# zkHubHQ/distributed-groth16

Measured on AMD Instinct MI355X. Metric: groth16_constraints_per_sec, higher is better.
Workload: dtype u32; 1 GPU; BN254 Groth16 prove from the matrices, synthetic R1CS with 2^20 - 2 constraints (3 nonzeros per row of A and B), 2^20 wires, 2 instance variables; r, s != 0 (R1CS x witness + 6 NTTs of 2^20 + 4 G1 MSMs + 1 G2 MSM); proving key RESIDENT as window tables (built once per key outside the timed region); curve=bn254, log_domain=20, parallelism=single GPU, key_table_bytes=6039807360, key_table_stride=1

## Files before the change

distributed-groth16_amd/csrc/ntt.hip:

```cpp
#include <cstdio>
#include <cstdlib>
#include "ctx.h"
#include "fp29.h"
#include "types.h"

namespace dg16 {

static void optional_table_skipped(const char* what, size_t bytes) {
  static const bool verbose = [] { const char* e = getenv("DG16_VERBOSE"); return e && atoi(e) != 0; }();
  if (verbose) fprintf(stderr, "[dg16] %s (%zu bytes) not built: hipMalloc failed; using the composed form\n", what, bytes);
}


constexpr unsigned kTileLog = 10;
constexpr unsigned kTile = 1u << kTileLog;
constexpr unsigned kMaxStepLog = 10;
constexpr unsigned kLoBits = 11;

template <class F>
struct StepArgs {
  const F* src[3];
  F* dst[3];
  unsigned log_n, s, log_a, log_b;
  unsigned last;
  unsigned log_n1, log_n2;
  const F* small;
  unsigned sm;
  const F* tw_lo;
  const F* tw_hi;
  unsigned lb;
  const F* tw_full;
  const F* post_full;
  const F* pre_lo;
  const F* pre_hi;
  const F* post_lo;
  const F* post_hi;
  unsigned plb;
  const F* scale;
  unsigned src_piece_log, dst_piece_log;
  size_t src_piece_stride, dst_piece_stride;
};

__device__ __forceinline__ unsigned bitrev(unsigned v, unsigned bits) {
  return bits ? (__brev(v) >> (32 - bits)) : 0;
}

constexpr int kNttBound = 48 * 64;
constexpr int kNttIn = 128;
constexpr int kNttFirstOut = 9 * 64;
constexpr int kNttStepGrowth = 6 * 64 + 32;
constexpr int kNttOddGrowth = 3 * 64 + 32;
static_assert(kNttFirstOut + (int)((kMaxStepLog - 2) / 2) * kNttStepGrowth + kNttOddGrowth <= kNttBound,
              "NTT tile bound: a pass of kMaxStepLog levels can exceed kNttBound");

template <class F>
__global__ void __launch_bounds__(256) ntt_step_kernel(StepArgs<F> p) {
  using P = typename F::Params;
  using T = RR<P>;
  constexpr int N = T::N;
  using El = Fe<P, kNttBound, 1>;
  using Tw = Fe<P, 64, 1>;
  __shared__ uint32_t tile_w[kTile * N];
  constexpr int NLW = T::NL;
  __shared__ uint32_t tw_w[(1u << (kMaxStepLog - 1)) * NLW];
  static_assert((1u << (kMaxStepLog - 2)) * N <= (1u << (kMaxStepLog - 1)) * NLW, "unpacked twiddles of the shorter steps fit");
  const unsigned tid = threadIdx.x;
  const unsigned s = p.s;
  const unsigned nj = 1u << s;
  const unsigned log_t = (p.log_n < kTileLog ? p.log_n : kTileLog) - s;
  const unsigned Tn = 1u << log_t;
  const unsigned elems = nj << log_t;
  const size_t tile_id = blockIdx.x;
  auto slot = [](unsigned e) { return (e ^ ((e >> 2) & 31u)) * (unsigned)N; };
  auto ld_tile = [&](unsigned i) {
    El v;
    const unsigned o = slot(i);
#pragma unroll
    for (int j = 0; j < N; j++) v.l[j] = tile_w[o + j];
    return v;
  };
  auto st_tile = [&](unsigned i, const El& v) {
    const unsigned o = slot(i);
#pragma unroll
    for (int j = 0; j < N; j++) tile_w[o + j] = v.l[j];
  };
  const bool tw_packed = p.s == kMaxStepLog;
  auto ld_tw = [&](unsigned i) {
    if (tw_packed) return fe_from_words<P>(&tw_w[i * NLW]);
    Tw v;
#pragma unroll
    for (int j = 0; j < N; j++) v.l[j] = tw_w[i * N + j];
    return v;
  };
  auto ld_packed = [&](const F* ptr) { return fe_from_words<P>(ptr->l); };

  size_t a = 0, b0 = 0, k1_0 = 0, k2 = 0;
  if (!p.last) {
    const unsigned tiles_per_a_log = p.log_b - log_t;
    a = tile_id >> tiles_per_a_log;
    b0 = (tile_id & (((size_t)1 << tiles_per_a_log) - 1)) << log_t;
  } else {
    const unsigned k1_tiles_log = p.log_n1 - log_t;
    k2 = tile_id >> k1_tiles_log;
    k1_0 = (tile_id & (((size_t)1 << k1_tiles_log) - 1)) << log_t;
  }

  if (s >= 1)
    for (unsigned t = tid; t < (nj >> 1); t += 256) {
      const F* w = p.small + ((size_t)t << (p.sm - s));
      if (tw_packed) {
#pragma unroll
        for (int j = 0; j < NLW; j++) tw_w[t * NLW + j] = w->l[j];
      } else {
        const Tw u = ld_packed(w);
#pragma unroll
        for (int j = 0; j < N; j++) tw_w[t * N + j] = u.l[j];
      }
    }

  for (unsigned idx = tid; idx < elems; idx += 256) {
    unsigned n, t;
    size_t g;
    if (!p.last) {
      t = idx & (Tn - 1);
      n = idx >> log_t;
      g = ((((a << s) + n) << p.log_b) + b0 + t);
    } else {
      n = idx & (nj - 1);
      t = idx >> s;
      g = ((((k1_0 + t) << p.log_n2) + k2) << s) + n;
    }
    const size_t gs = p.src_piece_stride ? (g >> p.src_piece_log) * p.src_piece_stride + (g & (((size_t)1 << p.src_piece_log) - 1)) : g;
    const Tw x = ld_packed(p.src[blockIdx.y] + gs);
    El v = x.template as<kNttBound, 1>();
    if (p.pre_lo) {
      const auto w = ld_packed(p.pre_lo + (g & ((1u << p.plb) - 1))) * ld_packed(p.pre_hi + (g >> p.plb));
      v = (x * w).template as<kNttBound, 1>();
    }
    st_tile((bitrev(n, s) << log_t) + t, v);
  }
  __syncthreads();

  unsigned lv = 1;
  if (s >= 2) {
    using In = Fe<P, kNttIn, 1>;
    const Tw w3 = ld_tw(1u << (s - 2));
    for (unsigned q = tid; q < (elems >> 2); q += 256) {
      const unsigned t = q & (Tn - 1), pi = q >> log_t;
      const unsigned ia = (pi << (2 + log_t)) + t;
      const In xa = ld_tile(ia).template unsafe_assume<kNttIn, 1>(), xb = ld_tile(ia + Tn).template unsafe_assume<kNttIn, 1>(),
               xc = ld_tile(ia + 2 * Tn).template unsafe_assume<kNttIn, 1>(), xd = ld_tile(ia + 3 * Tn).template unsafe_assume<kNttIn, 1>();
      const auto a1 = xa + xb;
      const auto b1 = xa - xb;
      const auto c1 = xc + xd;
      const auto te = (xc - xd) * w3;
      const auto o0 = a1 + c1;
      const auto o2 = a1 - c1;
      const auto o1 = b1 + te;
      const auto o3 = b1 - te;
      static_assert(decltype(o0)::Bound <= kNttFirstOut && decltype(o1)::Bound <= kNttFirstOut &&
                    decltype(o2)::Bound <= kNttFirstOut && decltype(o3)::Bound <= kNttFirstOut, "first radix-4 step bound");
      st_tile(ia, norm(o0).template as<kNttBound, 1>());
      st_tile(ia + 2 * Tn, norm(o2).template as<kNttBound, 1>());
      st_tile(ia + Tn, norm(o1).template as<kNttBound, 1>());
      st_tile(ia + 3 * Tn, norm(o3).template as<kNttBound, 1>());
    }
    __syncthreads();
    lv = 3;
  }
  for (; lv + 1 <= s; lv += 2) {
    const unsigned half = 1u << (lv - 1);
    const unsigned sh1 = s - lv, sh2 = s - lv - 1;
    for (unsigned q = tid; q < (elems >> 2); q += 256) {
      const unsigned t = q & (Tn - 1), pi = q >> log_t;
      const unsigned k = pi & (half - 1), blk = pi >> (lv - 1);
      const unsigned ia = ((((blk << (lv + 1)) + k)) << log_t) + t;
      const unsigned st = half << log_t;
      const El xa = ld_tile(ia), xb = ld_tile(ia + st), xc = ld_tile(ia + 2 * st), xd = ld_tile(ia + 3 * st);
      const Tw w1 = ld_tw(k << sh1);
      const auto tb = xb * w1;
      const auto td = xd * w1;
      const auto a1 = xa + tb;
      const auto b1 = xa - tb;
      const auto c1 = xc + td;
      const auto d1 = xc - td;
      const auto tc = c1 * ld_tw(k << sh2);
      const auto te = d1 * ld_tw((k + half) << sh2);
      const auto o0 = a1 + tc;
      const auto o2 = a1 - tc;
      const auto o1 = b1 + te;
      const auto o3 = b1 - te;
      static_assert(decltype(o0)::Bound - kNttBound <= kNttStepGrowth && decltype(o1)::Bound - kNttBound <= kNttStepGrowth &&
                    decltype(o2)::Bound - kNttBound <= kNttStepGrowth && decltype(o3)::Bound - kNttBound <= kNttStepGrowth,
                    "radix-4 step growth");
      st_tile(ia, norm(o0).template unsafe_assume<kNttBound, 1>());
      st_tile(ia + 2 * st, norm(o2).template unsafe_assume<kNttBound, 1>());
      st_tile(ia + st, norm(o1).template unsafe_assume<kNttBound, 1>());
      st_tile(ia + 3 * st, norm(o3).template unsafe_assume<kNttBound, 1>());
    }
    __syncthreads();
  }
  if (lv == s) {
    const unsigned half = 1u << (s - 1);
    for (unsigned q = tid; q < (elems >> 1); q += 256) {
      const unsigned t = q & (Tn - 1), k = q >> log_t;
      const unsigned i0 = (k << log_t) + t, i1 = i0 + (half << log_t);
      const El x = ld_tile(i0);
      const auto ty = ld_tile(i1) * ld_tw(k);
      const auto o0 = x + ty;
      const auto o1 = x - ty;
      static_assert(decltype(o0)::Bound - kNttBound <= kNttOddGrowth && decltype(o1)::Bound - kNttBound <= kNttOddGrowth,
                    "odd level growth");
      st_tile(i0, norm(o0).template unsafe_assume<kNttBound, 1>());
      st_tile(i1, norm(o1).template unsafe_assume<kNttBound, 1>());
    }
    __syncthreads();
  }

  for (unsigned idx = tid; idx < elems; idx += 256) {
    unsigned t = idx & (Tn - 1);
    unsigned k = idx >> log_t;
    const El v = ld_tile((k << log_t) + t);
    Fe<P, 64, 1> out;
    size_t g;
    if (!p.last) {
      size_t b = b0 + t;
      size_t e = (b * k) << p.log_a;
      if (p.tw_full) {
        if (e || p.scale) out = canon(v * ld_packed(p.tw_full + (((size_t)k << p.log_b) + b)));
        else out = canon(v);
      } else if (e) {
        const auto w = ld_packed(p.tw_lo + (e & ((1u << p.lb) - 1))) * ld_packed(p.tw_hi + (e >> p.lb));
        out = canon(v * w);
      } else if (p.scale) {
        out = canon(v * ld_packed(p.tw_hi));
      } else {
        out = canon(v);
      }
      g = ((((a << s) + k) << p.log_b) + b);
    } else {
      g = (k1_0 + t) + (k2 << p.log_n1) + ((size_t)k << (p.log_n1 + p.log_n2));
      if (p.post_full) {
        const auto w = ld_packed(p.post_full + g);
        if (p.scale) out = canon((v * ld_packed(p.scale)) * w);
        else out = canon(v * w);
      } else if (p.scale && p.post_lo) {
        const auto w = ld_packed(p.post_lo + (g & ((1u << p.plb) - 1))) * ld_packed(p.post_hi + (g >> p.plb));
        out = canon((v * ld_packed(p.scale)) * w);
      } else if (p.scale) {
        out = canon(v * ld_packed(p.scale));
      } else if (p.post_lo) {
        const auto w = ld_packed(p.post_lo + (g & ((1u << p.plb) - 1))) * ld_packed(p.post_hi + (g >> p.plb));
        out = canon(v * w);
      } else {
        out = canon(v);
      }
    }
    F o;
    fe_to_words<P>(out, o.l);
    if (p.dst_piece_stride) g = (g >> p.dst_piece_log) * p.dst_piece_stride + (g & (((size_t)1 << p.dst_piece_log) - 1));
    p.dst[blockIdx.y][g] = o;
  }
}

template <class F>
__global__ void to_internal_kernel(F* t, size_t count) {
  size_t j = (size_t)blockIdx.x * blockDim.x + threadIdx.x;
  if (j >= count) return;
  using P = typename F::Params;
  F c;
#pragma unroll
  for (int i = 0; i < F::NL; i++) c.l[i] = RR<P>::R_WORDS.v[i];
  t[j] = t[j] * c;
}
template <class F>
static void* internal_copy(hipStream_t s, const void* src, size_t count) {
  void* d = nullptr;
  DG_HIP(hipMalloc(&d, count * sizeof(F)));
  DG_HIP(hipMemcpyAsync(d, src, count * sizeof(F), hipMemcpyDeviceToDevice, s));
  hipLaunchKernelGGL(to_internal_kernel<F>, dim3((unsigned)((count + 255) / 256)), dim3(256), 0, s, (F*)d, count);
  return d;
}

template <class F>
__global__ void powers_kernel(F* out, size_t count, unsigned shift, const F* base_ptr,
                              unsigned root_log, int invert, const F* c_ptr) {
  size_t j = (size_t)blockIdx.x * blockDim.x + threadIdx.x;
  if (j >= count) return;
  F base;
  if (base_ptr) {
    base = *base_ptr;
  } else {
    F w;
#pragma unroll
    for (int i = 0; i < F::NL; i++) w.l[i] = F::Params::TWO_ADIC_ROOT[i];
    for (unsigned i = root_log; i < (unsigned)F::Params::TWO_ADICITY; i++) w = w.sqr();
    if (invert) {
      F acc = F::one(), sq = w;
      for (unsigned i = 0; i < root_log; i++) { acc = acc * sq; sq = sq.sqr(); }
      w = acc;
    }
    base = w;
  }
  F r = base.pow_u64((uint64_t)j << shift);
  if (c_ptr) r = r * *c_ptr;
  out[j] = r;
}

template <class F>
__global__ void n_inv_kernel(F* out, unsigned log_n) {
  F two = F::one() + F::one();
  F half = two.inv();
  *out = half.pow_u64(log_n);
}

struct Plan {
  unsigned nsteps;
  unsigned s[3];
};
static Plan make_plan(unsigned log_n) {
  Plan pl{};
  if (log_n <= kTileLog && log_n <= kMaxStepLog) {
    pl.nsteps = 1;
    pl.s[0] = log_n;
  } else if (log_n <= 2 * kMaxStepLog) {
    pl.nsteps = 2;
    pl.s[0] = log_n / 2;
    pl.s[1] = log_n - pl.s[0];
  } else {
    pl.nsteps = 3;
    pl.s[0] = log_n / 3;
    pl.s[1] = (log_n - pl.s[0]) / 2;
    pl.s[2] = log_n - pl.s[0] - pl.s[1];
  }
  return pl;
}

constexpr unsigned kFullTwiddleMaxLog = 24;
inline unsigned full_twiddle_min_log() {
  static const unsigned v = [] { const char* e = getenv("DG16_NTT_TABLE_MIN_LOG"); return e ? (unsigned)atoi(e) : 21u; }();
  return v;
}
template <class F>
__global__ void __launch_bounds__(256) full_twiddle_kernel(F* __restrict__ out, size_t count, unsigned log_a, unsigned log_b,
                                                            const F* __restrict__ lo, const F* __restrict__ hi, unsigned lb) {
  using P = typename F::Params;
  const size_t idx = (size_t)blockIdx.x * blockDim.x + threadIdx.x;
  if (idx >= count) return;
  const size_t k = idx >> log_b, b = idx & (((size_t)1 << log_b) - 1);
  const size_t e = (b * k) << log_a;
  const auto w = fe_from_words<P>(lo[e & (((size_t)1 << lb) - 1)].l) * fe_from_words<P>(hi[e >> lb].l);
  F o;
  fe_to_words<P>(canon(w), o.l);
  out[idx] = o;
}
template <class F>
__global__ void __launch_bounds__(256) flat_powers_kernel(F* __restrict__ out, size_t count, const F* __restrict__ lo,
                                                           const F* __restrict__ hi, unsigned lb) {
  using P = typename F::Params;
  const size_t o = (size_t)blockIdx.x * blockDim.x + threadIdx.x;
  if (o >= count) return;
  const auto w = fe_from_words<P>(lo[o & (((size_t)1 << lb) - 1)].l) * fe_from_words<P>(hi[o >> lb].l);
  F r;
  fe_to_words<P>(canon(w), r.l);
  out[o] = r;
}

template <class F>
static const TwiddleSet& get_twiddles(Call& k, int curve, unsigned log_n, int inverse) {
  std::lock_guard<std::mutex> g(k.ctx->mu);
  TwiddleKey key{curve, log_n, inverse};
  auto it = k.ctx->twiddles.find(key);
  if (it != k.ctx->twiddles.end()) return it->second;
  TwiddleSet ts;
  ts.lb = log_n < kLoBits ? log_n : kLoBits;
  ts.sm = log_n < kMaxStepLog ? (log_n ? log_n : 1) : kMaxStepLog;
  size_t nlo = (size_t)1 << ts.lb, nhi = (size_t)1 << (log_n - ts.lb), nsm = (size_t)1 << (ts.sm - 1);
  DG_HIP(hipMalloc(&ts.lo, nlo * sizeof(F)));
  DG_HIP(hipMalloc(&ts.hi, nhi * sizeof(F)));
  DG_HIP(hipMalloc(&ts.small, nsm * sizeof(F)));
  DG_HIP(hipMalloc(&ts.n_inv, sizeof(F)));
  hipStream_t s = k.s();
  hipLaunchKernelGGL(n_inv_kernel<F>, dim3(1), dim3(1), 0, s, (F*)ts.n_inv, log_n);
  hipLaunchKernelGGL(powers_kernel<F>, dim3((unsigned)((nlo + 255) / 256)), dim3(256), 0, s, (F*)ts.lo,
                     nlo, 0u, (const F*)nullptr, log_n, inverse, (const F*)nullptr);
  hipLaunchKernelGGL(powers_kernel<F>, dim3((unsigned)((nhi + 255) / 256)), dim3(256), 0, s, (F*)ts.hi,
                     nhi, ts.lb, (const F*)nullptr, log_n, inverse, (const F*)nullptr);
  if (inverse) {
    DG_HIP(hipMalloc(&ts.hi_scaled, nhi * sizeof(F)));
    hipLaunchKernelGGL(powers_kernel<F>, dim3((unsigned)((nhi + 255) / 256)), dim3(256), 0, s,
                       (F*)ts.hi_scaled, nhi, ts.lb, (const F*)nullptr, log_n, inverse,
                       (const F*)ts.n_inv);
  }
  hipLaunchKernelGGL(powers_kernel<F>, dim3((unsigned)((nsm + 255) / 256)), dim3(256), 0, s, (F*)ts.small,
                     nsm, log_n >= ts.sm ? log_n - ts.sm : 0, (const F*)nullptr, log_n ? log_n : 1, inverse,
                     (const F*)nullptr);
  ts.lo_i = internal_copy<F>(s, ts.lo, nlo);
  ts.hi_i = internal_copy<F>(s, ts.hi, nhi);
  if (inverse) ts.hi_scaled_i = internal_copy<F>(s, ts.hi_scaled, nhi);
  ts.small_i = internal_copy<F>(s, ts.small, nsm);
  ts.n_inv_i = internal_copy<F>(s, ts.n_inv, 1);
  {
    const Plan pl = make_plan(log_n);
    unsigned consumed = 0;
    for (unsigned j = 0; j + 1 < pl.nsteps && log_n <= kFullTwiddleMaxLog && log_n >= full_twiddle_min_log(); j++) {
      const size_t cnt = (size_t)1 << (log_n - consumed);
      if (hipMalloc(&ts.full[j], cnt * sizeof(F)) != hipSuccess) {
        (void)hipGetLastError();
        ts.full[j] = nullptr;
        optional_table_skipped("inter-step twiddle table", cnt * sizeof(F));
        consumed += pl.s[j];
        continue;
      }
      hipLaunchKernelGGL(full_twiddle_kernel<F>, dim3((unsigned)((cnt + 255) / 256)), dim3(256), 0, s, (F*)ts.full[j], cnt,
                         consumed, log_n - consumed - pl.s[j], (const F*)ts.lo_i,
                         (const F*)((inverse && j == 0) ? ts.hi_scaled_i : ts.hi_i), ts.lb);
      consumed += pl.s[j];
    }
  }
  DG_HIP(hipGetLastError());
  DG_HIP(hipStreamSynchronize(s));
  return k.ctx->twiddles.emplace(key, ts).first->second;
}

template <class F>
static void build_power_tables(Call& k, const F* g_dev, unsigned log_n, F* lo, F* hi, unsigned lb) {
  size_t nlo = (size_t)1 << lb, nhi = (size_t)1 << (log_n - lb);
  hipLaunchKernelGGL(powers_kernel<F>, dim3((unsigned)((nlo + 255) / 256)), dim3(256), 0, k.s(), lo, nlo, 0u,
                     g_dev, 0u, 0, (const F*)nullptr);
  hipLaunchKernelGGL(powers_kernel<F>, dim3((unsigned)((nhi + 255) / 256)), dim3(256), 0, k.s(), hi, nhi, lb,
                     g_dev, 0u, 0, (const F*)nullptr);
  hipLaunchKernelGGL(to_internal_kernel<F>, dim3((unsigned)((nlo + 255) / 256)), dim3(256), 0, k.s(), lo, nlo);
  hipLaunchKernelGGL(to_internal_kernel<F>, dim3((unsigned)((nhi + 255) / 256)), dim3(256), 0, k.s(), hi, nhi);
  DG_HIP(hipGetLastError());
}

template <class F>
__global__ void inv_one_kernel(F* out, const F* in) { *out = in->inv(); }

template <class F>
static void ntt_run_batch(Call& k, int curve, unsigned nb, const F* const* in, F* const* data, F* const* tmp,
                          unsigned log_n, int inverse, const F* pre_lo, const F* pre_hi, const F* post_lo,
                          const F* post_hi, unsigned plb, unsigned src_piece_log = 0, size_t src_piece_stride = 0,
                          unsigned dst_piece_log = 0, size_t dst_piece_stride = 0, const F* post_full = nullptr) {
  DG_REQUIRE(log_n <= 3 * kMaxStepLog, DG16_ERR_UNSUPPORTED, "log_n > 27 not supported yet");
  DG_REQUIRE(nb >= 1 && nb <= 3, DG16_ERR_BAD_ARG, "1..3 transforms per batch");
  const TwiddleSet& ts = get_twiddles<F>(k, curve, log_n, inverse);
  Plan pl = make_plan(log_n);
  unsigned consumed = 0;
  for (unsigned j = 0; j < pl.nsteps; j++) {
    StepArgs<F> a{};
    a.log_n = log_n;
    a.s = pl.s[j];
    a.log_a = consumed;
    a.log_b = log_n - consumed - pl.s[j];
    a.last = (j == pl.nsteps - 1);
    a.log_n1 = pl.nsteps >= 2 ? pl.s[0] : 0;
    a.log_n2 = pl.nsteps == 3 ? pl.s[1] : 0;
    a.small = (const F*)ts.small_i;
    a.sm = ts.sm;
    a.tw_lo = (const F*)ts.lo_i;
    bool fold_scale = inverse && pl.nsteps > 1 && j == 0;
    a.tw_hi = (const F*)(fold_scale ? ts.hi_scaled_i : ts.hi_i);
    a.lb = ts.lb;
    a.tw_full = (!a.last && j < 2) ? (const F*)ts.full[j] : nullptr;
    a.scale = nullptr;
    if (fold_scale) a.scale = (const F*)ts.n_inv_i;
    if (inverse && pl.nsteps == 1) a.scale = (const F*)ts.n_inv_i;
    if (j == 0) { a.pre_lo = pre_lo; a.pre_hi = pre_hi; a.src_piece_log = src_piece_log; a.src_piece_stride = src_piece_stride; }
    if (a.last) { a.post_lo = post_lo; a.post_hi = post_hi; a.post_full = post_full; a.dst_piece_log = dst_piece_log; a.dst_piece_stride = dst_piece_stride; }
    a.plb = plb;
    for (unsigned i = 0; i < nb; i++) {
      a.src[i] = j == 0 ? in[i] : tmp[i];
      a.dst[i] = (pl.nsteps == 1 || a.last) ? data[i] : tmp[i];
    }
    unsigned log_tile = log_n < kTileLog ? log_n : kTileLog;
    size_t blocks = (size_t)1 << (log_n - log_tile);
    if (a.last && pl.nsteps > 1) {
      unsigned log_t = log_tile - a.s;
      DG_REQUIRE(a.log_n1 >= log_t, DG16_ERR_UNSUPPORTED, "plan violates N1 >= T");
    } else if (!a.last) {
      unsigned log_t = log_tile - a.s;
      DG_REQUIRE(a.log_b >= log_t, DG16_ERR_UNSUPPORTED, "plan violates B >= T");
    }
    hipLaunchKernelGGL(ntt_step_kernel<F>, dim3((unsigned)blocks, nb), dim3(256), 0, k.s(), a);
    DG_HIP(hipGetLastError());
    consumed += pl.s[j];
  }
}
template <class F>
static void ntt_run(Call& k, int curve, F* data, F* tmp, unsigned log_n, int inverse,
                    const F* pre_lo, const F* pre_hi, const F* post_lo, const F* post_hi, unsigned plb) {
  const F* in[1] = {data};
  F* d[1] = {data};
  F* t[1] = {tmp};
  ntt_run_batch<F>(k, curve, 1, in, d, t, log_n, inverse, pre_lo, pre_hi, post_lo, post_hi, plb);
}

template <class F>
static void ntt_typed(Call& k, int curve, void* data, unsigned log_n, int inverse, const void* coset_host) {
  F* d = (F*)data;
  F* tmp = (F*)ws(k.c, 8, sizeof(F) << log_n);
  const F *pre_lo = nullptr, *pre_hi = nullptr, *post_lo = nullptr, *post_hi = nullptr;
  unsigned plb = log_n < kLoBits ? log_n : kLoBits;
  if (coset_host) {
    F* g = (F*)ws(k.c, 9, 2 * sizeof(F));
    DG_HIP(hipMemcpyAsync(g, coset_host, sizeof(F), hipMemcpyHostToDevice, k.s()));
    F* lo = (F*)ws(k.c, 10, sizeof(F) << plb);
    F* hi = (F*)ws(k.c, 11, sizeof(F) << (log_n - plb));
    if (inverse) {
      hipLaunchKernelGGL(inv_one_kernel<F>, dim3(1), dim3(1), 0, k.s(), g + 1, g);
      build_power_tables<F>(k, g + 1, log_n, lo, hi, plb);
      post_lo = lo; post_hi = hi;
    } else {
      build_power_tables<F>(k, g, log_n, lo, hi, plb);
      pre_lo = lo; pre_hi = hi;
    }
  }
  k.begin_dominant();
  ntt_run<F>(k, curve, d, tmp, log_n, inverse, pre_lo, pre_hi, post_lo, post_hi, plb);
  k.end_dominant();
}

const TwiddleSet& get_twiddles_any(Call& k, int curve, unsigned log_n, int inverse) {
  switch (curve) {
    case 0: return get_twiddles<bn254_fr>(k, curve, log_n, inverse);
    case 1: return get_twiddles<bls12_381_fr>(k, curve, log_n, inverse);
    default: return get_twiddles<bls12_377_fr>(k, curve, log_n, inverse);
  }
}

void ntt_launch(Call& k, int curve, void* data, unsigned log_n, int inverse, const void* coset_host) {
  switch (curve) {
    case 0: ntt_typed<bn254_fr>(k, curve, data, log_n, inverse, coset_host); break;
    case 1: ntt_typed<bls12_381_fr>(k, curve, data, log_n, inverse, coset_host); break;
    default: ntt_typed<bls12_377_fr>(k, curve, data, log_n, inverse, coset_host); break;
  }
}

template <class F>
__global__ void __launch_bounds__(256) mul_sub_kernel(const F* __restrict__ a, const F* __restrict__ b,
                                                       const F* __restrict__ c, F* __restrict__ out, size_t n) {
  size_t stride = (size_t)gridDim.x * blockDim.x;
  for (size_t i = (size_t)blockIdx.x * blockDim.x + threadIdx.x; i < n; i += stride)
    out[i] = a[i] * b[i] - c[i];
}

template <class F>
static const F* flat_shift_table(Call& k, const TwiddleSet& t2, unsigned log_m) {
  std::lock_guard<std::mutex> g(k.ctx->mu);
  TwiddleSet& w = const_cast<TwiddleSet&>(t2);
  if (!w.shift_full && !w.shift_full_tried) {
    w.shift_full_tried = true;
    const size_t m = (size_t)1 << log_m;
    if (hipMalloc(&w.shift_full, m * sizeof(F)) != hipSuccess) {
      (void)hipGetLastError();
      w.shift_full = nullptr;
      optional_table_skipped("w_2m shift table", m * sizeof(F));
      return nullptr;
    }
    hipLaunchKernelGGL(flat_powers_kernel<F>, dim3((unsigned)((m + 255) / 256)), dim3(256), 0, k.s(), (F*)w.shift_full, m,
                       (const F*)t2.lo_i, (const F*)t2.hi_i, t2.lb);
    DG_HIP(hipGetLastError());
    DG_HIP(hipStreamSynchronize(k.s()));
  }
  return (const F*)w.shift_full;
}

template <class F>
static void h_poly_typed(Call& k, int curve, const void* a, const void* b, const void* c, unsigned log_m,
                         void* out) {
  size_t bytes = sizeof(F) << log_m;
  F* v[3] = {(F*)ws(k.c, 12, bytes), (F*)ws(k.c, 13, bytes), (F*)ws(k.c, 14, bytes)};
  F* t0 = (F*)ws(k.c, 8, 3 * bytes);
  F* tmp[3] = {t0, t0 + ((size_t)1 << log_m), t0 + ((size_t)2 << log_m)};
  const F* in[3] = {(const F*)a, (const F*)b, (const F*)c};
  const TwiddleSet& t2 = get_twiddles<F>(k, curve, log_m + 1, 0);
  const F* shift = log_m <= kFullTwiddleMaxLog && log_m >= full_twiddle_min_log() ? flat_shift_table<F>(k, t2, log_m) : nullptr;
  k.begin_dominant();
  ntt_run_batch<F>(k, curve, 3, in, v, tmp, log_m, 1, nullptr, nullptr, (const F*)t2.lo_i, (const F*)t2.hi_i, t2.lb,
                   0, 0, 0, 0, shift);
  ntt_run_batch<F>(k, curve, 3, v, v, tmp, log_m, 0, nullptr, nullptr, nullptr, nullptr, 0);
  size_t n = (size_t)1 << log_m;
  size_t blocks = (n + 255) / 256;
  size_t cap = (size_t)k.ctx->compute_units * 8;
  if (blocks > cap) blocks = cap;
  hipLaunchKernelGGL(mul_sub_kernel<F>, dim3((unsigned)blocks), dim3(256), 0, k.s(), v[0], v[1], v[2], (F*)out, n);
  DG_HIP(hipGetLastError());
  k.end_dominant();
}


template <class F>
__device__ __forceinline__ F tw_lookup(const F* lo, const F* hi, unsigned lb, size_t e) {
  const size_t l = e & (((size_t)1 << lb) - 1), h = e >> lb;
  if (l == 0) return hi[h];
  if (h == 0) return lo[l];
  return lo[l] * hi[h];
}

template <int LOGN, class F>
__device__ __forceinline__ void small_dft(F* x, const F* roots) {
  constexpr int N = 1 << LOGN;
#pragma unroll
  for (int i = 0; i < N; i++) {
    int j = 0;
#pragma unroll
    for (int b = 0; b < LOGN; b++) j |= ((i >> b) & 1) << (LOGN - 1 - b);
    if (j > i) { const F t = x[i]; x[i] = x[j]; x[j] = t; }
  }
#pragma unroll
  for (int lv = 1; lv <= LOGN; lv++) {
    constexpr int dummy = 0; (void)dummy;
    const int half = 1 << (lv - 1);
#pragma unroll
    for (int q = 0; q < N / 2; q++) {
      const int kk = q & (half - 1), blk = q >> (lv - 1);
      const int i0 = (blk << lv) + kk, i1 = i0 + half;
      const F y = kk ? x[i1] * roots[kk << (LOGN - lv)] : x[i1];
      const F u = x[i0];
      x[i0] = u + y;
      x[i1] = u - y;
    }
  }
}

struct CrossArgs {
  const void *wi_lo, *wi_hi, *wf_lo, *wf_hi, *g_lo, *g_hi, *n_inv;
  unsigned wlb, glb;
  unsigned log_m, rank;
  size_t S;
};

template <class F, int LOGN>
__global__ void __launch_bounds__(256) hdist_cross_kernel(const F* __restrict__ in, F* __restrict__ out, CrossArgs p) {
  constexpr int N = 1 << LOGN;
  const size_t j = (size_t)blockIdx.x * blockDim.x + threadIdx.x;
  if (j >= p.S) return;
  const unsigned v = blockIdx.y;
  const size_t M = p.S << LOGN;
  const size_t k2 = (size_t)p.rank * p.S + j;
  const F *wi_lo = (const F*)p.wi_lo, *wi_hi = (const F*)p.wi_hi, *wf_lo = (const F*)p.wf_lo, *wf_hi = (const F*)p.wf_hi;
  const F *g_lo = (const F*)p.g_lo, *g_hi = (const F*)p.g_hi;
  F x[N];
#pragma unroll
  for (int i = 0; i < N; i++) x[i] = in[((size_t)i * 3 + v) * p.S + j];
  {
    const F base = tw_lookup(wi_lo, wi_hi, p.wlb, k2);
    F pw = base;
#pragma unroll
    for (int i = 1; i < N; i++) {
      x[i] = x[i] * pw;
      if (i + 1 < N) pw = pw * base;
    }
  }
  F roots[N / 2 ? N / 2 : 1];
#pragma unroll
  for (int t = 0; t < N / 2; t++) roots[t] = tw_lookup(wi_lo, wi_hi, p.wlb, M * t);
  small_dft<LOGN>(x, roots);
  {
    const F gm = tw_lookup(g_lo, g_hi, p.glb, M);
    F pw = tw_lookup(g_lo, g_hi, p.glb, k2) * *(const F*)p.n_inv;
#pragma unroll
    for (int i = 0; i < N; i++) {
      x[i] = x[i] * pw;
      if (i + 1 < N) pw = pw * gm;
    }
  }
#pragma unroll
  for (int t = 0; t < N / 2; t++) roots[t] = tw_lookup(wf_lo, wf_hi, p.wlb, M * t);
  small_dft<LOGN>(x, roots);
  {
    const F base = tw_lookup(wf_lo, wf_hi, p.wlb, k2);
    F pw = base;
#pragma unroll
    for (int i = 1; i < N; i++) {
      x[i] = x[i] * pw;
      if (i + 1 < N) pw = pw * base;
    }
  }
#pragma unroll
  for (int i = 0; i < N; i++) out[((size_t)i * 3 + v) * p.S + j] = x[i];
}

template <class F, int LOGN>
__global__ void __launch_bounds__(256) ntt_dist_cross_kernel(const F* __restrict__ in, F* __restrict__ out, const F* w_lo,
                                                              const F* w_hi, unsigned wlb, const F* n_inv, unsigned rank,
                                                              size_t S) {
  constexpr int N = 1 << LOGN;
  const size_t j = (size_t)blockIdx.x * blockDim.x + threadIdx.x;
  if (j >= S) return;
  const size_t M = S << LOGN, k2 = (size_t)rank * S + j;
  F x[N];
#pragma unroll
  for (int i = 0; i < N; i++) x[i] = in[(size_t)i * S + j];
  {
    const F base = tw_lookup(w_lo, w_hi, wlb, k2);
    F pw = base;
#pragma unroll
    for (int i = 1; i < N; i++) {
      x[i] = x[i] * pw;
      if (i + 1 < N) pw = pw * base;
    }
  }
  F roots[N / 2 ? N / 2 : 1];
#pragma unroll
  for (int t = 0; t < N / 2; t++) roots[t] = tw_lookup(w_lo, w_hi, wlb, M * t);
  small_dft<LOGN>(x, roots);
#pragma unroll
  for (int i = 0; i < N; i++) out[(size_t)i * S + j] = n_inv ? x[i] * *n_inv : x[i];
}

static unsigned log2_exact(unsigned n) {
  unsigned l = 0;
  while ((1u << l) < n) l++;
  DG_REQUIRE((1u << l) == n, DG16_ERR_BAD_ARG, "rank count must be a power of two");
  return l;
}

template <class F>
static void h_poly_dist_stage_typed(Call& k, int curve, unsigned log_m, unsigned rank, unsigned n_ranks, int stage,
                                    const void* const* in, void* out) {
  const unsigned log_n = log2_exact(n_ranks);
  DG_REQUIRE(log_n >= 1 && log_n <= 3, DG16_ERR_UNSUPPORTED, "sharded h-polynomial: 2, 4 or 8 ranks");
  DG_REQUIRE(log_m >= 2 * log_n, DG16_ERR_BAD_ARG, "sharded h-polynomial: domain smaller than ranks^2");
  DG_REQUIRE(rank < n_ranks, DG16_ERR_BAD_ARG, "rank out of range");
  const unsigned log_M = log_m - log_n, log_S = log_M - log_n;
  const size_t M = (size_t)1 << log_M, S = (size_t)1 << log_S;
  F* t0 = (F*)ws(k.c, 8, 3 * M * sizeof(F));
  F* tmp[3] = {t0, t0 + M, t0 + 2 * M};
  if (stage == 0) {
    const F* src[3] = {(const F*)in[0], (const F*)in[1], (const F*)in[2]};
    F* dst[3] = {(F*)out, (F*)out + S, (F*)out + 2 * S};
    ntt_run_batch<F>(k, curve, 3, src, dst, tmp, log_M, 1, nullptr, nullptr, nullptr, nullptr, 0, 0, 0, log_S, 3 * S);
  } else if (stage == 1) {
    const TwiddleSet& wi = get_twiddles<F>(k, curve, log_m, 1);
    const TwiddleSet& wf = get_twiddles<F>(k, curve, log_m, 0);
    const TwiddleSet& g = get_twiddles<F>(k, curve, log_m + 1, 0);
    const TwiddleSet& nn = get_twiddles<F>(k, curve, log_n, 1);
    CrossArgs a{wi.lo, wi.hi, wf.lo, wf.hi, g.lo, g.hi, nn.n_inv, wi.lb, g.lb, log_m, rank, S};
    dim3 grid((unsigned)((S + 255) / 256), 3);
    switch (log_n) {
      case 1: hipLaunchKernelGGL((hdist_cross_kernel<F, 1>), grid, dim3(256), 0, k.s(), (const F*)in[0], (F*)out, a); break;
      case 2: hipLaunchKernelGGL((hdist_cross_kernel<F, 2>), grid, dim3(256), 0, k.s(), (const F*)in[0], (F*)out, a); break;
      default: hipLaunchKernelGGL((hdist_cross_kernel<F, 3>), grid, dim3(256), 0, k.s(), (const F*)in[0], (F*)out, a); break;
    }
    DG_HIP(hipGetLastError());
  } else {
    const F* base = (const F*)in[0];
    const F* src[3] = {base, base + S, base + 2 * S};
    F* v0 = (F*)ws(k.c, 12, 3 * M * sizeof(F));
    F* v[3] = {v0, v0 + M, v0 + 2 * M};
    ntt_run_batch<F>(k, curve, 3, src, v, tmp, log_M, 0, nullptr, nullptr, nullptr, nullptr, 0, log_S, 3 * S, 0, 0);
    size_t blocks = (M + 255) / 256;
    size_t cap = (size_t)k.ctx->compute_units * 8;
    if (blocks > cap) blocks = cap;
    hipLaunchKernelGGL(mul_sub_kernel<F>, dim3((unsigned)blocks), dim3(256), 0, k.s(), v[0], v[1], v[2], (F*)out, M);
    DG_HIP(hipGetLastError());
  }
}

template <class F>
static void ntt_dist_stage_typed(Call& k, int curve, unsigned log_n_total, unsigned rank, unsigned n_ranks, int inverse,
                                 int stage, const void* in, void* out) {
  const unsigned log_n = log2_exact(n_ranks);
  DG_REQUIRE(log_n >= 1 && log_n <= 3, DG16_ERR_UNSUPPORTED, "sharded NTT: 2, 4 or 8 ranks");
  DG_REQUIRE(log_n_total >= 2 * log_n, DG16_ERR_BAD_ARG, "sharded NTT: domain smaller than ranks^2");
  DG_REQUIRE(rank < n_ranks, DG16_ERR_BAD_ARG, "rank out of range");
  const unsigned log_M = log_n_total - log_n;
  const size_t M = (size_t)1 << log_M, S = M >> log_n;
  if (stage == 0) {
    F* tmp = (F*)ws(k.c, 8, M * sizeof(F));
    const F* src[1] = {(const F*)in};
    F* dst[1] = {(F*)out};
    F* t[1] = {tmp};
    ntt_run_batch<F>(k, curve, 1, src, dst, t, log_M, inverse, nullptr, nullptr, nullptr, nullptr, 0);
  } else {
    const TwiddleSet& w = get_twiddles<F>(k, curve, log_n_total, inverse);
    const F* n_inv = inverse ? (const F*)get_twiddles<F>(k, curve, log_n, 1).n_inv : nullptr;
    dim3 grid((unsigned)((S + 255) / 256));
#define DG_NDX(L)                                                                                                   \
  hipLaunchKernelGGL((ntt_dist_cross_kernel<F, L>), grid, dim3(256), 0, k.s(), (const F*)in, (F*)out, (const F*)w.lo, \
                     (const F*)w.hi, w.lb, n_inv, rank, S)
    switch (log_n) {
      case 1: DG_NDX(1); break;
      case 2: DG_NDX(2); break;
      default: DG_NDX(3); break;
    }
#undef DG_NDX
    DG_HIP(hipGetLastError());
  }
}
void ntt_dist_stage(Call& k, int curve, unsigned log_n_total, unsigned rank, unsigned n_ranks, int inverse, int stage,
                    const void* in, void* out) {
  switch (curve) {
    case 0: ntt_dist_stage_typed<bn254_fr>(k, curve, log_n_total, rank, n_ranks, inverse, stage, in, out); break;
    case 1: ntt_dist_stage_typed<bls12_381_fr>(k, curve, log_n_total, rank, n_ranks, inverse, stage, in, out); break;
    default: ntt_dist_stage_typed<bls12_377_fr>(k, curve, log_n_total, rank, n_ranks, inverse, stage, in, out); break;
  }
}
void ntt_dist_launch(Call& k, int curve, const dg16_comm* comm, const void* in, void* out, unsigned log_n_total,
                     int inverse) {
  const unsigned n = comm->n_ranks(comm->self), rank = comm->rank(comm->self);
  const size_t bytes = (((size_t)1 << log_n_total) / n) * 32;
  void* buf_a = ws(k.c, 26, bytes);
  void* buf_b = ws(k.c, 27, bytes);
  ntt_dist_stage(k, curve, log_n_total, rank, n, inverse, 0, in, buf_a);
  int rc = comm->all_to_all(comm->self, buf_a, buf_b, bytes / n, k.s());
  DG_REQUIRE(rc == DG16_OK, DG16_ERR_NET, "all-to-all of the sharded NTT failed");
  ntt_dist_stage(k, curve, log_n_total, rank, n, inverse, 1, buf_b, out);
}

void h_poly_dist_stage(Call& k, int curve, unsigned log_m, unsigned rank, unsigned n_ranks, int stage,
                       const void* const* in, void* out) {
  switch (curve) {
    case 0: h_poly_dist_stage_typed<bn254_fr>(k, curve, log_m, rank, n_ranks, stage, in, out); break;
    case 1: h_poly_dist_stage_typed<bls12_381_fr>(k, curve, log_m, rank, n_ranks, stage, in, out); break;
    default: h_poly_dist_stage_typed<bls12_377_fr>(k, curve, log_m, rank, n_ranks, stage, in, out); break;
  }
}

void h_poly_dist_launch(Call& k, int curve, const dg16_comm* comm, const void* a, const void* b, const void* c,
                        unsigned log_m, void* out) {
  const unsigned n = comm->n_ranks(comm->self), rank = comm->rank(comm->self);
  const size_t M = ((size_t)1 << log_m) / n, bytes = 3 * M * 32;
  void* buf_a = ws(k.c, 26, bytes);
  void* buf_b = ws(k.c, 27, bytes);
  const void* rows[3] = {a, b, c};
  h_poly_dist_stage(k, curve, log_m, rank, n, 0, rows, buf_a);
  int rc = comm->all_to_all(comm->self, buf_a, buf_b, bytes / n, k.s());
  DG_REQUIRE(rc == DG16_OK, DG16_ERR_NET, "all-to-all of the sharded h-polynomial failed");
  const void* in1[1] = {buf_b};
  h_poly_dist_stage(k, curve, log_m, rank, n, 1, in1, buf_a);
  rc = comm->all_to_all(comm->self, buf_a, buf_b, bytes / n, k.s());
  DG_REQUIRE(rc == DG16_OK, DG16_ERR_NET, "all-to-all of the sharded h-polynomial failed");
  h_poly_dist_stage(k, curve, log_m, rank, n, 2, in1, out);
}

void h_poly_launch(Call& k, int curve, const void* a, const void* b, const void* c, unsigned log_m, void* out) {
  switch (curve) {
    case 0: h_poly_typed<bn254_fr>(k, curve, a, b, c, log_m, out); break;
    case 1: h_poly_typed<bls12_381_fr>(k, curve, a, b, c, log_m, out); break;
    default: h_poly_typed<bls12_377_fr>(k, curve, a, b, c, log_m, out); break;
  }
}

}
```

Measured before the change: 103.9 million constraints/s.

## Fuse last inverse NTT step with first forward NTT step in h-polynomial

Adds a kernel that runs the final inverse-NTT pass, applies the coset shift, and runs the first forward-NTT pass on the same shared-memory tile. The intermediate array therefore makes no round trip through global memory. To make the tiles line up, the inverse plan's step order is reversed. Shared kernel code is factored into helpers, and the fused path is on by default behind an environment flag. The costs are extra register pressure from holding a tile in registers between passes, and reversed-plan twiddle tables that may not be resident.

Measured after the change: 104.6 million constraints/s, median of 6. Within noise of the previous version (+0.6%).

```diff
diff --git a/distributed-groth16_amd/csrc/ntt.hip b/distributed-groth16_amd/csrc/ntt.hip
--- a/distributed-groth16_amd/csrc/ntt.hip
+++ b/distributed-groth16_amd/csrc/ntt.hip
@@ -53,94 +53,66 @@
 static_assert(kNttFirstOut + (int)((kMaxStepLog - 2) / 2) * kNttStepGrowth + kNttOddGrowth <= kNttBound,
               "NTT tile bound: a pass of kMaxStepLog levels can exceed kNttBound");
 
-template <class F>
-__global__ void __launch_bounds__(256) ntt_step_kernel(StepArgs<F> p) {
+template <class P>
+using NttEl = Fe<P, kNttBound, 1>;
+template <class P>
+using NttTw = Fe<P, 64, 1>;
+
+template <class P>
+__device__ __forceinline__ unsigned tile_slot(unsigned e) { return (e ^ ((e >> 2) & 31u)) * (unsigned)RR<P>::N; }
+template <class P>
+__device__ __forceinline__ NttEl<P> tile_ld(const uint32_t* tile_w, unsigned i) {
+  NttEl<P> v;
+  const unsigned o = tile_slot<P>(i);
+#pragma unroll
+  for (int j = 0; j < RR<P>::N; j++) v.l[j] = tile_w[o + j];
+  return v;
+}
+template <class P>
+__device__ __forceinline__ void tile_st(uint32_t* tile_w, unsigned i, const NttEl<P>& v) {
+  const unsigned o = tile_slot<P>(i);
+#pragma unroll
+  for (int j = 0; j < RR<P>::N; j++) tile_w[o + j] = v.l[j];
+}
+template <class P>
+__device__ __forceinline__ NttTw<P> tw_ld(const uint32_t* tw_w, bool tw_packed, unsigned i) {
+  if (tw_packed) return fe_from_words<P>(&tw_w[i * RR<P>::NL]);
+  NttTw<P> v;
+#pragma unroll
+  for (int j = 0; j < RR<P>::N; j++) v.l[j] = tw_w[i * RR<P>::N + j];
+  return v;
+}
+
+template <class F>
+__device__ __forceinline__ void ntt_stage_twiddles(uint32_t* tw_w, const F* small, unsigned sm, unsigned s, bool tw_packed) {
   using P = typename F::Params;
-  using T = RR<P>;
-  constexpr int N = T::N;
-  using El = Fe<P, kNttBound, 1>;
-  using Tw = Fe<P, 64, 1>;
-  __shared__ uint32_t tile_w[kTile * N];
-  constexpr int NLW = T::NL;
-  __shared__ uint32_t tw_w[(1u << (kMaxStepLog - 1)) * NLW];
-  static_assert((1u << (kMaxStepLog - 2)) * N <= (1u << (kMaxStepLog - 1)) * NLW, "unpacked twiddles of the shorter steps fit");
+  constexpr int N = RR<P>::N, NLW = RR<P>::NL;
   const unsigned tid = threadIdx.x;
-  const unsigned s = p.s;
-  const unsigned nj = 1u << s;
-  const unsigned log_t = (p.log_n < kTileLog ? p.log_n : kTileLog) - s;
-  const unsigned Tn = 1u << log_t;
-  const unsigned elems = nj << log_t;
-  const size_t tile_id = blockIdx.x;
-  auto slot = [](unsigned e) { return (e ^ ((e >> 2) & 31u)) * (unsigned)N; };
-  auto ld_tile = [&](unsigned i) {
-    El v;
-    const unsigned o = slot(i);
-#pragma unroll
-    for (int j = 0; j < N; j++) v.l[j] = tile_w[o + j];
-    return v;
-  };
-  auto st_tile = [&](unsigned i, const El& v) {
-    const unsigned o = slot(i);
-#pragma unroll
-    for (int j = 0; j < N; j++) tile_w[o + j] = v.l[j];
-  };
-  const bool tw_packed = p.s == kMaxStepLog;
-  auto ld_tw = [&](unsigned i) {
-    if (tw_packed) return fe_from_words<P>(&tw_w[i * NLW]);
-    Tw v;
-#pragma unroll
-    for (int j = 0; j < N; j++) v.l[j] = tw_w[i * N + j];
-    return v;
-  };
-  auto ld_packed = [&](const F* ptr) { return fe_from_words<P>(ptr->l); };
-
-  size_t a = 0, b0 = 0, k1_0 = 0, k2 = 0;
-  if (!p.last) {
-    const unsigned tiles_per_a_log = p.log_b - log_t;
-    a = tile_id >> tiles_per_a_log;
-    b0 = (tile_id & (((size_t)1 << tiles_per_a_log) - 1)) << log_t;
-  } else {
-    const unsigned k1_tiles_log = p.log_n1 - log_t;
-    k2 = tile_id >> k1_tiles_log;
-    k1_0 = (tile_id & (((size_t)1 << k1_tiles_log) - 1)) << log_t;
-  }
-
   if (s >= 1)
-    for (unsigned t = tid; t < (nj >> 1); t += 256) {
-      const F* w = p.small + ((size_t)t << (p.sm - s));
+    for (unsigned t = tid; t < (1u << (s - 1)); t += 256) {
+      const F* w = small + ((size_t)t << (sm - s));
       if (tw_packed) {
 #pragma unroll
         for (int j = 0; j < NLW; j++) tw_w[t * NLW + j] = w->l[j];
       } else {
-        const Tw u = ld_packed(w);
+        const NttTw<P> u = fe_from_words<P>(w->l);
 #pragma unroll
         for (int j = 0; j < N; j++) tw_w[t * N + j] = u.l[j];
       }
     }
-
-  for (unsigned idx = tid; idx < elems; idx += 256) {
-    unsigned n, t;
-    size_t g;
-    if (!p.last) {
-      t = idx & (Tn - 1);
-      n = idx >> log_t;
-      g = ((((a << s) + n) << p.log_b) + b0 + t);
-    } else {
-      n = idx & (nj - 1);
-      t = idx >> s;
-      g = ((((k1_0 + t) << p.log_n2) + k2) << s) + n;
-    }
-    const size_t gs = p.src_piece_stride ? (g >> p.src_piece_log) * p.src_piece_stride + (g & (((size_t)1 << p.src_piece_log) - 1)) : g;
-    const Tw x = ld_packed(p.src[blockIdx.y] + gs);
-    El v = x.template as<kNttBound, 1>();
-    if (p.pre_lo) {
-      const auto w = ld_packed(p.pre_lo + (g & ((1u << p.plb) - 1))) * ld_packed(p.pre_hi + (g >> p.plb));
-      v = (x * w).template as<kNttBound, 1>();
-    }
-    st_tile((bitrev(n, s) << log_t) + t, v);
-  }
-  __syncthreads();
-
+}
+
+template <class P>
+__device__ __forceinline__ void ntt_tile_levels(uint32_t* tile_w, const uint32_t* tw_w, bool tw_packed, unsigned s,
+                                                unsigned log_t) {
+  using El = NttEl<P>;
+  using Tw = NttTw<P>;
+  const unsigned tid = threadIdx.x;
+  const unsigned Tn = 1u << log_t;
+  const unsigned elems = (1u << s) << log_t;
+  auto ld_tile = [&](unsigned i) { return tile_ld<P>(tile_w, i); };
+  auto st_tile = [&](unsigned i, const El& v) { tile_st<P>(tile_w, i, v); };
+  auto ld_tw = [&](unsigned i) { return tw_ld<P>(tw_w, tw_packed, i); };
   unsigned lv = 1;
   if (s >= 2) {
     using In = Fe<P, kNttIn, 1>;
@@ -216,6 +188,86 @@
     }
     __syncthreads();
   }
+}
+
+template <class F>
+__device__ __forceinline__ NttTw<typename F::Params> step_twiddled(const StepArgs<F>& p, const NttEl<typename F::Params>& v,
+                                                                   unsigned k, size_t b) {
+  using P = typename F::Params;
+  auto ld_packed = [](const F* ptr) { return fe_from_words<P>(ptr->l); };
+  const size_t e = (b * k) << p.log_a;
+  if (p.tw_full) {
+    if (e || p.scale) return canon(v * ld_packed(p.tw_full + (((size_t)k << p.log_b) + b)));
+    return canon(v);
+  }
+  if (e) {
+    const auto w = ld_packed(p.tw_lo + (e & ((1u << p.lb) - 1))) * ld_packed(p.tw_hi + (e >> p.lb));
+    return canon(v * w);
+  }
+  if (p.scale) return canon(v * ld_packed(p.tw_hi));
+  return canon(v);
+}
+
+template <class F>
+__global__ void __launch_bounds__(256) ntt_step_kernel(StepArgs<F> p) {
+  using P = typename F::Params;
+  using T = RR<P>;
+  constexpr int N = T::N;
+  using El = NttEl<P>;
+  using Tw = NttTw<P>;
+  __shared__ uint32_t tile_w[kTile * N];
+  constexpr int NLW = T::NL;
+  __shared__ uint32_t tw_w[(1u << (kMaxStepLog - 1)) * NLW];
+  static_assert((1u << (kMaxStepLog - 2)) * N <= (1u << (kMaxStepLog - 1)) * NLW, "unpacked twiddles of the shorter steps fit");
+  const unsigned tid = threadIdx.x;
+  const unsigned s = p.s;
+  const unsigned nj = 1u << s;
+  const unsigned log_t = (p.log_n < kTileLog ? p.log_n : kTileLog) - s;
+  const unsigned Tn = 1u << log_t;
+  const unsigned elems = nj << log_t;
+  const size_t tile_id = blockIdx.x;
+  auto ld_tile = [&](unsigned i) { return tile_ld<P>(tile_w, i); };
+  auto st_tile = [&](unsigned i, const El& v) { tile_st<P>(tile_w, i, v); };
+  const bool tw_packed = p.s == kMaxStepLog;
+  auto ld_packed = [&](const F* ptr) { return fe_from_words<P>(ptr->l); };
+
+  size_t a = 0, b0 = 0, k1_0 = 0, k2 = 0;
+  if (!p.last) {
+    const unsigned tiles_per_a_log = p.log_b - log_t;
+    a = tile_id >> tiles_per_a_log;
+    b0 = (tile_id & (((size_t)1 << tiles_per_a_log) - 1)) << log_t;
+  } else {
+    const unsigned k1_tiles_log = p.log_n1 - log_t;
+    k2 = tile_id >> k1_tiles_log;
+    k1_0 = (tile_id & (((size_t)1 << k1_tiles_log) - 1)) << log_t;
+  }
+
+  ntt_stage_twiddles<F>(tw_w, p.small, p.sm, s, tw_packed);
+
+  for (unsigned idx = tid; idx < elems; idx += 256) {
+    unsigned n, t;
+    size_t g;
+    if (!p.last) {
+      t = idx & (Tn - 1);
+      n = idx >> log_t;
+      g = ((((a << s) + n) << p.log_b) + b0 + t);
+    } else {
+      n = idx & (nj - 1);
+      t = idx >> s;
+      g = ((((k1_0 + t) << p.log_n2) + k2) << s) + n;
+    }
+    const size_t gs = p.src_piece_stride ? (g >> p.src_piece_log) * p.src_piece_stride + (g & (((size_t)1 << p.src_piece_log) - 1)) : g;
+    const Tw x = ld_packed(p.src[blockIdx.y] + gs);
+    El v = x.template as<kNttBound, 1>();
+    if (p.pre_lo) {
+      const auto w = ld_packed(p.pre_lo + (g & ((1u << p.plb) - 1))) * ld_packed(p.pre_hi + (g >> p.plb));
+      v = (x * w).template as<kNttBound, 1>();
+    }
+    st_tile((bitrev(n, s) << log_t) + t, v);
+  }
+  __syncthreads();
+
+  ntt_tile_levels<P>(tile_w, tw_w, tw_packed, s, log_t);
 
   for (unsigned idx = tid; idx < elems; idx += 256) {
     unsigned t = idx & (Tn - 1);
@@ -225,18 +277,7 @@
     size_t g;
     if (!p.last) {
       size_t b = b0 + t;
-      size_t e = (b * k) << p.log_a;
-      if (p.tw_full) {
-        if (e || p.scale) out = canon(v * ld_packed(p.tw_full + (((size_t)k << p.log_b) + b)));
-        else out = canon(v);
-      } else if (e) {
-        const auto w = ld_packed(p.tw_lo + (e & ((1u << p.lb) - 1))) * ld_packed(p.tw_hi + (e >> p.lb));
-        out = canon(v * w);
-      } else if (p.scale) {
-        out = canon(v * ld_packed(p.tw_hi));
-      } else {
-        out = canon(v);
-      }
+      out = step_twiddled<F>(p, v, k, b);
       g = ((((a << s) + k) << p.log_b) + b);
     } else {
       g = (k1_0 + t) + (k2 << p.log_n1) + ((size_t)k << (p.log_n1 + p.log_n2));
@@ -260,6 +301,77 @@
     fe_to_words<P>(out, o.l);
     if (p.dst_piece_stride) g = (g >> p.dst_piece_log) * p.dst_piece_stride + (g & (((size_t)1 << p.dst_piece_log) - 1));
     p.dst[blockIdx.y][g] = o;
+  }
+}
+
+template <class F>
+__global__ void __launch_bounds__(256) ntt_inv_fwd_kernel(StepArgs<F> inv, StepArgs<F> fwd) {
+  using P = typename F::Params;
+  using T = RR<P>;
+  constexpr int N = T::N;
+  using El = NttEl<P>;
+  using Tw = NttTw<P>;
+  __shared__ uint32_t tile_w[kTile * N];
+  constexpr int NLW = T::NL;
+  __shared__ uint32_t tw_w[(1u << (kMaxStepLog - 1)) * NLW];
+  constexpr unsigned kPer = kTile / 256;
+  const unsigned tid = threadIdx.x;
+  const unsigned s = inv.s;
+  const unsigned log_t = kTileLog - s;
+  const unsigned Tn = 1u << log_t;
+  const size_t tile_id = blockIdx.x;
+  const bool tw_packed = s == kMaxStepLog;
+  auto ld_packed = [](const F* ptr) { return fe_from_words<P>(ptr->l); };
+
+  const unsigned k1_tiles_log = inv.log_n1 - log_t;
+  const size_t k2 = tile_id >> k1_tiles_log;
+  const size_t k1_0 = (tile_id & (((size_t)1 << k1_tiles_log) - 1)) << log_t;
+  const size_t b0 = tile_id << log_t;
+
+  ntt_stage_twiddles<F>(tw_w, inv.small, inv.sm, s, tw_packed);
+  for (unsigned idx = tid; idx < kTile; idx += 256) {
+    const unsigned n = idx & ((1u << s) - 1), t = idx >> s;
+    const size_t g = ((((k1_0 + t) << inv.log_n2) + k2) << s) + n;
+    tile_st<P>(tile_w, (bitrev(n, s) << log_t) + t, ld_packed(inv.src[blockIdx.y] + g).template as<kNttBound, 1>());
+  }
+  __syncthreads();
+  ntt_tile_levels<P>(tile_w, tw_w, tw_packed, s, log_t);
+
+  El r[kPer];
+#pragma unroll
+  for (unsigned i = 0; i < kPer; i++) {
+    const unsigned idx = tid + 256 * i;
+    const unsigned t = idx & (Tn - 1), k = idx >> log_t;
+    const El v = tile_ld<P>(tile_w, idx);
+    const size_t o = (k1_0 + t) + (k2 << inv.log_n1) + ((size_t)k << (inv.log_n1 + inv.log_n2));
+    if (inv.post_full) {
+      const auto x = v * ld_packed(inv.post_full + o);
+      static_assert(decltype(x)::Bound <= kNttIn, "shift product exceeds the first radix-4 step's input bound");
+      r[i] = x.template as<kNttBound, 1>();
+    } else {
+      const auto x = v * (ld_packed(inv.post_lo + (o & ((1u << inv.plb) - 1))) * ld_packed(inv.post_hi + (o >> inv.plb)));
+      static_assert(decltype(x)::Bound <= kNttIn, "shift product exceeds the first radix-4 step's input bound");
+      r[i] = x.template as<kNttBound, 1>();
+    }
+  }
+  __syncthreads();
+  ntt_stage_twiddles<F>(tw_w, fwd.small, fwd.sm, s, tw_packed);
+#pragma unroll
+  for (unsigned i = 0; i < kPer; i++) {
+    const unsigned idx = tid + 256 * i;
+    const unsigned t = idx & (Tn - 1), k = idx >> log_t;
+    tile_st<P>(tile_w, (bitrev(k, s) << log_t) + t, r[i]);
+  }
+  __syncthreads();
+  ntt_tile_levels<P>(tile_w, tw_w, tw_packed, s, log_t);
+
+  for (unsigned idx = tid; idx < kTile; idx += 256) {
+    const unsigned t = idx & (Tn - 1), k = idx >> log_t;
+    const size_t b = b0 + t;
+    const Tw out = step_twiddled<F>(fwd, tile_ld<P>(tile_w, idx), k, b);
+    F o;
+    fe_to_words<P>(out, o.l);
+    fwd.dst[blockIdx.y][((size_t)k << fwd.log_b) + b] = o;
   }
 }
 
@@ -439,6 +551,46 @@
 __global__ void inv_one_kernel(F* out, const F* in) { *out = in->inv(); }
 
 template <class F>
+static StepArgs<F> plan_step_args(const TwiddleSet& ts, const Plan& pl, unsigned j, unsigned log_n, int inverse, bool tables) {
+  unsigned consumed = 0;
+  for (unsigned i = 0; i < j; i++) consumed += pl.s[i];
+  StepArgs<F> a{};
+  a.log_n = log_n;
+  a.s = pl.s[j];
+  a.log_a = consumed;
+  a.log_b = log_n - consumed - pl.s[j];
+  a.last = (j == pl.nsteps - 1);
+  a.log_n1 = pl.nsteps >= 2 ? pl.s[0] : 0;
+  a.log_n2 = pl.nsteps == 3 ? pl.s[1] : 0;
+  a.small = (const F*)ts.small_i;
+  a.sm = ts.sm;
+  a.tw_lo = (const F*)ts.lo_i;
+  bool fold_scale = inverse && pl.nsteps > 1 && j == 0;
+  a.tw_hi = (const F*)(fold_scale ? ts.hi_scaled_i : ts.hi_i);
+  a.lb = ts.lb;
+  a.tw_full = (tables && !a.last && j < 2) ? (const F*)ts.full[j] : nullptr;
+  a.scale = nullptr;
+  if (fold_scale) a.scale = (const F*)ts.n_inv_i;
+  if (inverse && pl.nsteps == 1) a.scale = (const F*)ts.n_inv_i;
+  return a;
+}
+
+template <class F>
+static void launch_step(Call& k, const StepArgs<F>& a, unsigned nb, bool multi_step) {
+  unsigned log_tile = a.log_n < kTileLog ? a.log_n : kTileLog;
+  size_t blocks = (size_t)1 << (a.log_n - log_tile);
+  if (a.last && multi_step) {
+    unsigned log_t = log_tile - a.s;
+    DG_REQUIRE(a.log_n1 >= log_t, DG16_ERR_UNSUPPORTED, "plan violates N1 >= T");
+  } else if (!a.last) {
+    unsigned log_t = log_tile - a.s;
+    DG_REQUIRE(a.log_b >= log_t, DG16_ERR_UNSUPPORTED, "plan violates B >= T");
+  }
+  hipLaunchKernelGGL(ntt_step_kernel<F>, dim3((unsigned)blocks, nb), dim3(256), 0, k.s(), a);
+  DG_HIP(hipGetLastError());
+}
+
+template <class F>
 static void ntt_run_batch(Call& k, int curve, unsigned nb, const F* const* in, F* const* data, F* const* tmp,
                           unsigned log_n, int inverse, const F* pre_lo, const F* pre_hi, const F* post_lo,
                           const F* post_hi, unsigned plb, unsigned src_piece_log = 0, size_t src_piece_stride = 0,
@@ -447,26 +599,8 @@
   DG_REQUIRE(nb >= 1 && nb <= 3, DG16_ERR_BAD_ARG, "1..3 transforms per batch");
   const TwiddleSet& ts = get_twiddles<F>(k, curve, log_n, inverse);
   Plan pl = make_plan(log_n);
-  unsigned consumed = 0;
   for (unsigned j = 0; j < pl.nsteps; j++) {
-    StepArgs<F> a{};
-    a.log_n = log_n;
-    a.s = pl.s[j];
-    a.log_a = consumed;
-    a.log_b = log_n - consumed - pl.s[j];
-    a.last = (j == pl.nsteps - 1);
-    a.log_n1 = pl.nsteps >= 2 ? pl.s[0] : 0;
-    a.log_n2 = pl.nsteps == 3 ? pl.s[1] : 0;
-    a.small = (const F*)ts.small_i;
-    a.sm = ts.sm;
-    a.tw_lo = (const F*)ts.lo_i;
-    bool fold_scale = inverse && pl.nsteps > 1 && j == 0;
-    a.tw_hi = (const F*)(fold_scale ? ts.hi_scaled_i : ts.hi_i);
-    a.lb = ts.lb;
-    a.tw_full = (!a.last && j < 2) ? (const F*)ts.full[j] : nullptr;
-    a.scale = nullptr;
-    if (fold_scale) a.scale = (const F*)ts.n_inv_i;
-    if (inverse && pl.nsteps == 1) a.scale = (const F*)ts.n_inv_i;
+    StepArgs<F> a = plan_step_args<F>(ts, pl, j, log_n, inverse, true);
     if (j == 0) { a.pre_lo = pre_lo; a.pre_hi = pre_hi; a.src_piece_log = src_piece_log; a.src_piece_stride = src_piece_stride; }
     if (a.last) { a.post_lo = post_lo; a.post_hi = post_hi; a.post_full = post_full; a.dst_piece_log = dst_piece_log; a.dst_piece_stride = dst_piece_stride; }
     a.plb = plb;
@@ -474,18 +608,7 @@
       a.src[i] = j == 0 ? in[i] : tmp[i];
       a.dst[i] = (pl.nsteps == 1 || a.last) ? data[i] : tmp[i];
     }
-    unsigned log_tile = log_n < kTileLog ? log_n : kTileLog;
-    size_t blocks = (size_t)1 << (log_n - log_tile);
-    if (a.last && pl.nsteps > 1) {
-      unsigned log_t = log_tile - a.s;
-      DG_REQUIRE(a.log_n1 >= log_t, DG16_ERR_UNSUPPORTED, "plan violates N1 >= T");
-    } else if (!a.last) {
-      unsigned log_t = log_tile - a.s;
-      DG_REQUIRE(a.log_b >= log_t, DG16_ERR_UNSUPPORTED, "plan violates B >= T");
-    }
-    hipLaunchKernelGGL(ntt_step_kernel<F>, dim3((unsigned)blocks, nb), dim3(256), 0, k.s(), a);
-    DG_HIP(hipGetLastError());
-    consumed += pl.s[j];
+    launch_step<F>(k, a, nb, pl.nsteps > 1);
   }
 }
 template <class F>
@@ -567,6 +690,12 @@
   return (const F*)w.shift_full;
 }
 
+static bool hpoly_fuse_enabled() {
+  static const bool v = [] { const char* e = getenv("DG16_HPOLY_FUSE"); return !e || atoi(e) != 0; }();
+  return v;
+}
+static bool hpoly_fusable(const Plan& fp) { return fp.nsteps == 2 || (fp.nsteps == 3 && fp.s[0] == fp.s[2]); }
+
 template <class F>
 static void h_poly_typed(Call& k, int curve, const void* a, const void* b, const void* c, unsigned log_m,
                          void* out) {
@@ -577,15 +706,48 @@
   const F* in[3] = {(const F*)a, (const F*)b, (const F*)c};
   const TwiddleSet& t2 = get_twiddles<F>(k, curve, log_m + 1, 0);
   const F* shift = log_m <= kFullTwiddleMaxLog && log_m >= full_twiddle_min_log() ? flat_shift_table<F>(k, t2, log_m) : nullptr;
+  const Plan fp = make_plan(log_m);
+  const bool fuse = log_m <= 3 * kMaxStepLog && hpoly_fuse_enabled() && hpoly_fusable(fp);
+  F* const* h = v;
   k.begin_dominant();
-  ntt_run_batch<F>(k, curve, 3, in, v, tmp, log_m, 1, nullptr, nullptr, (const F*)t2.lo_i, (const F*)t2.hi_i, t2.lb,
-                   0, 0, 0, 0, shift);
-  ntt_run_batch<F>(k, curve, 3, v, v, tmp, log_m, 0, nullptr, nullptr, nullptr, nullptr, 0);
+  if (fuse) {
+    Plan ip = fp;
+    for (unsigned j = 0; j < fp.nsteps; j++) ip.s[j] = fp.s[fp.nsteps - 1 - j];
+    const bool ip_tables = ip.s[0] == fp.s[0] && ip.s[1] == fp.s[1];
+    const TwiddleSet& ti = get_twiddles<F>(k, curve, log_m, 1);
+    const TwiddleSet& tf = get_twiddles<F>(k, curve, log_m, 0);
+    for (unsigned j = 0; j + 1 < ip.nsteps; j++) {
+      StepArgs<F> st = plan_step_args<F>(ti, ip, j, log_m, 1, ip_tables);
+      for (unsigned i = 0; i < 3; i++) { st.src[i] = j == 0 ? in[i] : tmp[i]; st.dst[i] = tmp[i]; }
+      launch_step<F>(k, st, 3, true);
+    }
+    StepArgs<F> il = plan_step_args<F>(ti, ip, ip.nsteps - 1, log_m, 1, ip_tables);
+    il.post_full = shift;
+    il.post_lo = (const F*)t2.lo_i;
+    il.post_hi = (const F*)t2.hi_i;
+    il.plb = t2.lb;
+    StepArgs<F> f0 = plan_step_args<F>(tf, fp, 0, log_m, 0, true);
+    for (unsigned i = 0; i < 3; i++) { il.src[i] = tmp[i]; f0.dst[i] = v[i]; }
+    DG_REQUIRE(il.s == f0.s && il.log_n1 >= kTileLog - il.s && f0.log_b >= kTileLog - f0.s && !il.scale,
+               DG16_ERR_UNSUPPORTED, "h-polynomial: plans do not fuse");
+    hipLaunchKernelGGL(ntt_inv_fwd_kernel<F>, dim3((unsigned)((size_t)1 << (log_m - kTileLog)), 3), dim3(256), 0, k.s(), il, f0);
+    DG_HIP(hipGetLastError());
+    for (unsigned j = 1; j < fp.nsteps; j++) {
+      StepArgs<F> st = plan_step_args<F>(tf, fp, j, log_m, 0, true);
+      for (unsigned i = 0; i < 3; i++) { st.src[i] = v[i]; st.dst[i] = st.last ? tmp[i] : v[i]; }
+      launch_step<F>(k, st, 3, true);
+    }
+    h = tmp;
+  } else {
+    ntt_run_batch<F>(k, curve, 3, in, v, tmp, log_m, 1, nullptr, nullptr, (const F*)t2.lo_i, (const F*)t2.hi_i, t2.lb,
+                     0, 0, 0, 0, shift);
+    ntt_run_batch<F>(k, curve, 3, v, v, tmp, log_m, 0, nullptr, nullptr, nullptr, nullptr, 0);
+  }
   size_t n = (size_t)1 << log_m;
   size_t blocks = (n + 255) / 256;
   size_t cap = (size_t)k.ctx->compute_units * 8;
   if (blocks > cap) blocks = cap;
-  hipLaunchKernelGGL(mul_sub_kernel<F>, dim3((unsigned)blocks), dim3(256), 0, k.s(), v[0], v[1], v[2], (F*)out, n);
+  hipLaunchKernelGGL(mul_sub_kernel<F>, dim3((unsigned)blocks), dim3(256), 0, k.s(), h[0], h[1], h[2], (F*)out, n);
   DG_HIP(hipGetLastError());
   k.end_dominant();
 }
```
